# hpy666666/ChineseChessAI

Measured on AMD Instinct MI355X. Metric: self-play games/sec @ 50 MCTS sims, higher is better.
Workload: dtype bf16

## Files before the change

chinesechessai_amd/_lib.py:

```python
import ctypes as C
import os
import subprocess
import sys

_HERE = os.path.dirname(os.path.abspath(__file__))
CSRC = os.path.join(_HERE, "csrc")
LIB_PATH = os.path.join(CSRC, "libxq_hip.so")
SOURCES = [os.path.join(CSRC, "xq_engine.hip"), os.path.join(CSRC, "xq_conv.hip"), os.path.join(CSRC, "xq_replay.hip"),
           os.path.join(CSRC, "xq_tower.hip"), os.path.join(CSRC, "xq_policy.hip")]
HEADERS = [os.path.join(CSRC, "xq_device.hpp"), os.path.join(CSRC, "xq_attack.hpp"), os.path.join(CSRC, "xq_mfma.hpp"), os.path.join(CSRC, "xq_tower_probes.hpp"),
           os.path.join(CSRC, "xq_tower1wa.hpp"), os.path.join(CSRC, "xq_tower1wa_body.inc"), os.path.join(CSRC, "xq_policy_fc1w_body.inc"),
           os.path.join(_HERE, "..", "include", "xq_selfplay.h"), os.path.join(_HERE, "..", "include", "xq_debug.h")]

MAX_MOVES = 128
MAX_PLIES = 70
WINNER_NONE = 2
NO_KING = -1
POLICY_SIZE = 8100
STATE_WORDS = 10
(S_PLAYER, S_MOVE_COUNT, S_WINNER, S_RED_KING, S_BLACK_KING, S_NO_CAPTURE, S_CONSEC_CHECKS, S_REASON,
 S_REASON_SIDE, S_REASON_COUNT) = range(10)
EVAL_PRIORS, EVAL_LOGITS_F32, EVAL_LOGITS_BF16 = 0, 1, 2
PLANES_NONE, PLANES_NCHW_F32, PLANES_NCHW_BF16, PLANES_NHWC16_BF16 = 0, 1, 2, 3
SAMPLE_RECORD_BYTES = 48 + 8 + 4 + 4 + 256 + 256
# ... 98 lines not shown
                                     C.c_void_p, C.c_void_p, C.c_void_p]),
    "xq_engine_create": (C.c_int, [C.POINTER(Config), C.POINTER(C.c_void_p)]),
    "xq_engine_destroy": (None, [C.c_void_p]),
    "xq_engine_set_stream": (C.c_int, [C.c_void_p, C.c_void_p]),
    "xq_engine_set_pow_table": (C.c_int, [C.c_void_p, C.c_void_p, C.c_int]),
    "xq_engine_new_games": (C.c_int, [C.c_void_p, C.c_void_p]),
    "xq_engine_set_logit_columns": (C.c_int, [C.c_void_p, C.c_void_p, C.c_int]),
    "xq_engine_set_temperature": (C.c_int, [C.c_void_p, C.c_double, C.c_void_p, C.c_int]),
    "xq_engine_set_root_noise": (C.c_int, [C.c_void_p, C.c_double, C.c_double, C.c_uint64]),
    "xq_engine_set_tree_reuse": (C.c_int, [C.c_void_p, C.c_int]),
    "xq_engine_set_virtual_loss": (C.c_int, [C.c_void_p, C.c_int]),
    "xq_engine_leaf_slots": (C.c_int, [C.c_void_p]),
    "xq_engine_tree_stats": (C.c_int, [C.c_void_p, C.c_void_p, C.c_void_p]),
    "xq_engine_read_root_priors": (C.c_int, [C.c_void_p, C.c_void_p]),
    "xq_engine_set_uniforms": (C.c_int, [C.c_void_p, C.c_void_p]),
    "xq_engine_set_roots": (C.c_int, [C.c_void_p, C.c_void_p, C.c_void_p]),
    "xq_engine_search_round": (C.c_int, [C.c_void_p, C.c_int, C.c_int, C.c_void_p, C.c_void_p, C.c_void_p]),
    "xq_engine_eval_hashnet": (C.c_int, [C.c_void_p, C.c_int]),
    "xq_engine_end_search": (C.c_int, [C.c_void_p, C.c_int, C.c_void_p, C.c_void_p]),
    "xq_engine_play_move": (C.c_int, [C.c_void_p]),
    "xq_engine_finalize": (C.c_int, [C.c_void_p]),
    "xq_engine_active_games": (C.c_int, [C.c_void_p, C.c_void_p]),
    "xq_engine_active_games_post": (C.c_int, [C.c_void_p]),
    "xq_engine_active_games_poll": (C.c_int, [C.c_void_p, C.c_void_p, C.c_void_p]),
    "xq_engine_priors_ptr": (C.c_void_p, [C.c_void_p]),
    "xq_engine_values_ptr": (C.c_void_p, [C.c_void_p]),
    "xq_engine_rounds_per_move": (C.c_int, [C.c_void_p]),
    "xq_engine_read_leaves": (C.c_int, [C.c_void_p] * 6),
    "xq_engine_write_priors": (C.c_int, [C.c_void_p] * 3),
    "xq_engine_read_root_visits": (C.c_int, [C.c_void_p] * 4),
    "xq_engine_read_tree": (C.c_int, [C.c_void_p, C.c_int, C.c_int] + [C.c_void_p] * 8),
    "xq_engine_read_games": (C.c_int, [C.c_void_p] * 8),
    "xq_engine_read_samples": (C.c_int, [C.c_void_p] * 9),
    "xq_engine_pack_samples": (C.c_int, [C.c_void_p, C.c_void_p]),
    "xq_engine_set_root_eval_carry": (C.c_int, [C.c_void_p, C.c_int]),
    "xq_engine_roots_not_ready": (C.c_int, [C.c_void_p, C.c_void_p]),
    "xq_engine_set_row_compaction": (C.c_int, [C.c_void_p, C.c_int]),
    "xq_engine_set_leaf_dedupe": (C.c_int, [C.c_void_p, C.c_int]),
    "xq_engine_set_eval_cache": (C.c_int, [C.c_void_p, C.c_int]),
    "xq_engine_eval_cache_stats": (C.c_int, [C.c_void_p, C.c_void_p, C.c_int]),
    "xq_engine_row_map": (C.c_int, [C.c_void_p, C.POINTER(C.c_void_p), C.POINTER(C.c_void_p)]),
    "xq_engine_read_row_history": (C.c_int, [C.c_void_p, C.c_void_p, C.c_int, C.POINTER(C.c_int64), C.c_int]),
    "xq_engine_read_leaf_rows": (C.c_int, [C.c_void_p, C.c_void_p]),
    "xq_engine_refill_begin": (C.c_int, [C.c_void_p, C.c_void_p, C.c_int]),
    "xq_engine_refill_step": (C.c_int, [C.c_void_p, C.c_void_p, C.c_void_p]),
    "xq_engine_refill_read_games": (C.c_int, [C.c_void_p] * 8),
    "xq_engine_refill_read_slots": (C.c_int, [C.c_void_p, C.c_void_p]),
    "xq_engine_set_pairing": (C.c_int, [C.c_void_p, C.c_void_p]),
    "xq_engine_refill_begin2": (C.c_int, [C.c_void_p, C.c_void_p, C.c_int, C.c_void_p]),
    "xq_engine_search_round2": (C.c_int, [C.c_void_p, C.c_int, C.c_int, C.c_void_p, C.c_void_p, C.c_int, C.c_void_p, C.c_void_p,
                                          C.c_void_p]),
    "xq_engine_end_search2": (C.c_int, [C.c_void_p, C.c_int, C.c_void_p, C.c_void_p, C.c_int, C.c_void_p, C.c_void_p]),
    "xq_engine_row_map_net": (C.c_int, [C.c_void_p, C.c_int, C.POINTER(C.c_void_p), C.POINTER(C.c_void_p)]),
    "xq_engine_read_row_history_net": (C.c_int, [C.c_void_p, C.c_int, C.c_void_p, C.c_int, C.POINTER(C.c_int64), C.c_int]),
    "xq_engine_eval_hashnet2": (C.c_int, [C.c_void_p, C.c_int, C.c_int]),
    "xq_engine_set_per_slot_reuse": (C.c_int, [C.c_void_p, C.c_int, C.c_int]),
    "xq_conv3x3_nhwc_bf16": (C.c_int, [C.c_void_p, C.c_void_p, C.c_void_p, C.c_void_p, C.c_void_p, C.c_void_p,
                                       C.c_int, C.c_int, C.c_int]),
    "xq_heads_nhwc_bf16": (C.c_int, [C.c_void_p] * 6 + [C.c_int]),
    "xq_tower_nhwc_bf16": (C.c_int, [C.c_void_p] * 9 + [C.c_int, C.c_int, C.c_void_p, C.c_void_p]),
    "xq_policy_fc_bf16": (C.c_int, [C.c_void_p] * 5 + [C.c_int, C.c_int, C.c_int, C.c_void_p]),
    "xq_value_head_bf16": (C.c_int, [C.c_void_p] * 7 + [C.c_int, C.c_void_p]),
    "xq_replay_last_error": (C.c_char_p, []),
    "xq_replay_create": (C.c_int, [C.c_int, C.c_int64, C.POINTER(C.c_void_p)]),
    "xq_replay_destroy": (None, [C.c_void_p]),
    "xq_replay_size": (C.c_int64, [C.c_void_p]),
    "xq_replay_push_records": (C.c_int, [C.c_void_p, C.c_void_p, C.c_void_p, C.c_int, C.c_void_p]),
    "xq_replay_encode_batch": (C.c_int, [C.c_void_p, C.c_void_p, C.c_void_p, C.c_int, C.c_void_p, C.c_void_p]),
    "xq_replay_read_records": (C.c_int, [C.c_void_p, C.c_void_p, C.c_void_p, C.c_int, C.c_void_p]),
    "xq_engine_profile": (C.c_int, [C.c_void_p, C.c_int]),
    "xq_engine_profile_read": (C.c_int, [C.c_void_p] * 5),
}

_DEBUG_SIGNATURES = {
    "xq_tower_set_variant": (None, [C.c_int]),
    "xq_tower_set_clock_sample": (None, [C.c_void_p]),
    "xq_tower_debug_stamps": (C.c_int, [C.c_void_p] * 9 + [C.c_int, C.c_int, C.c_void_p]),
    "xq_mfma_probe": (C.c_int, [C.c_void_p] * 4 + [C.c_int, C.c_int, C.c_int]),
    "xq_conv3x3_set_variant": (None, [C.c_int]),
    "xq_conv3x3_debug_stamps": (C.c_int, [C.c_int, C.c_int] + [C.c_void_p] * 6 + [C.c_int, C.c_int, C.c_void_p]),
    "xq_engine_set_search_occupancy": (None, [C.c_int]),
    "xq_engine_set_search_stamps": (C.c_int, [C.c_void_p]),
    "xq_policy_fc_set_variant": (None, [C.c_int]),
    "xq_policy_fc_debug_stamps": (C.c_int, [C.c_int, C.c_void_p, C.c_void_p, C.c_void_p, C.c_void_p, C.c_void_p, C.c_int, C.c_int, C.c_int, C.c_void_p]),
    "xq_policy_fc_debug": (C.c_int, [C.c_int] + [C.c_void_p] * 5 + [C.c_int, C.c_int, C.c_int]),
}

EXPORTS = sorted(_SIGNATURES)
DEBUG_EXPORTS = sorted(_DEBUG_SIGNATURES)
ROW_HISTORY = 65536


def lib():
    global _lib
    if _lib is None:
        if not os.path.exists(LIB_PATH):
            try:
                build()
            except Exception as ex:
                raise XqError("libxq_hip.so is not built (%s) and could not be compiled (%s): run "
                              "`python -c 'import __graft_entry__ as g; g.build()'`; the HIP path has no CPU fallback"
                              % (LIB_PATH, ex))
        _preload_torch_hip_runtime()
        L = C.CDLL(LIB_PATH)
        for table in (_SIGNATURES, _DEBUG_SIGNATURES):
            for name, (res, args) in table.items():
                fn = getattr(L, name)
                fn.restype = res
                fn.argtypes = args
        _lib = L
    return _lib


def check(rc):
    if rc != 0:
        msg = lib().xq_last_error()
        raise XqError("libxq_hip error %d: %s" % (rc, msg.decode() if msg else "?"))


def ptr(a):
    return None if a is None else a.ctypes.data_as(C.c_void_p)
```

chinesechessai_amd/csrc/xq_engine.hip:

```cpp
#include "xq_device.hpp"
#include "../../include/xq_selfplay.h"
#include "../../include/xq_debug.h"
#include <hip/hip_runtime.h>
#include <math.h>
#include <stdio.h>
#include <stdlib.h>
#include <string.h>
#include <string>
#include <thread>
#include <vector>

using namespace xq;

struct __align__(16) GameS {
    int8_t  side;
    uint8_t move_count;
    int8_t  winner;
    uint8_t reason;
    int8_t  reason_side;
    uint8_t reason_count;
    int8_t  rk, bk;
    uint8_t nocap, cchk, n_hist, n_root;
    uint8_t done, n_samples, error, n_plies;
};
// ... 1083 lines not shown
                    if (lane == 0) E.leaf_side[slot] = (int8_t)leaf_side;
                    if (lane == 1) E.leaf_net[slot] = (uint8_t)net;
                }
                if (planes) write_planes(bd, leaf_side, planes, fmt, slot);
            };
            const MoveResult mr = wave_make_move<false, true>(L.bd, st, L.path_move[depth - 1], hist, L.maps, L.cand, L.legal, L.own_sq,
                                                              early, E.want_check != 0);
            flags |= mr.is_check ? F_CHECK : 0;
            XQ_STAMP(7);
            const bool terminal = (mr.n_legal == 0) || (st.winner != WINNER_NONE);
            if (!terminal) {
                if (lane == 0) {
                    T.fl[node] = (uint8_t)flags;
                    E.leaf_node[slot] = (uint16_t)node; E.leaf_mult[slot] = (uint8_t)sims_left; E.leaf_n[slot] = (uint8_t)mr.n_legal;
                    E.leaf_depth[slot] = (uint8_t)depth;
                }
                for (int j = lane; j < mr.n_legal; j += 64) E.leaf_moves[(size_t)slot * MAXM + j] = L.legal[j];
                if (lane < depth) E.leaf_path[(size_t)slot * PATH_CAP + lane] = L.path_node[lane];
                if (depth > 64 && lane + 64 < depth) E.leaf_path[(size_t)slot * PATH_CAP + 64 + lane] = L.path_node[lane + 64];
                if (STAMP && lane == 0) stp[8] = __builtin_amdgcn_s_memtime();
                const uint32_t bdw = lane < 12 ? pack_dword(L.bd, lane) : 0u;
                int ec = -1;
                if (E.ec_on) {
                    ec = eval_cache_probe(E, h, bdw, leaf_side, net, ec_first, true, E.dedupe && (unsigned)(look.ent >> 32) == E.dd_tag);
                    if (lane == 0) E.leaf_ec[slot] = ec;
                }
                if (E.dedupe && (ec < 0 || E.ec_on == 2)) dedupe_finish(E, slot, bdw, leaf_side, look, net);
                if (STAMP && lane == 0) stp[9] = __builtin_amdgcn_s_memtime();
                return;
            }
            flags |= F_TERM;
            if (st.winner == st.side) flags |= F_VAL_POS;
            else if (st.winner == -st.side) flags |= F_VAL_NEG;
            if (lane == 0) T.fl[node] = (uint8_t)flags;
        }
        const double v = (flags & F_VAL_POS) ? 1.0 : ((flags & F_VAL_NEG) ? -1.0 : 0.0);
        backup(T, root, L.path_node, depth, v, 1);
        sims_left--;
    }
}

template <int OCC, bool VL, bool STAMP = false>
__global__ __launch_bounds__(64, OCC) void k_search_round(Eng E, int round, int batch_count, EvalPair ev, void *planes, int fmt,
                                                          unsigned long long *stamps = nullptr)
{
    __shared__ WaveLds L;
    if constexpr (VL) search_round_generic<true>(E, L, round, batch_count, ev, planes, fmt);
    else search_round_one<STAMP>(E, L, round, batch_count, ev, planes, fmt, stamps);
}

__constant__ uint32_t c_crc_table[256];

__device__ __forceinline__ uint32_t crc_byte(uint32_t crc, uint32_t b)
{
    return c_crc_table[(crc ^ b) & 0xffu] ^ (crc >> 8);
}

__global__ __launch_bounds__(64) void k_hashnet(Eng E, int salt0, int salt1)
{
    __shared__ WaveLds L;
    const int g = blockIdx.x, lane = XQ_LANE;
    if (E.gs[g / E.leaf_slots].done || E.leaf_node[g] == LEAF_NONE) return;
    unpack_to_lds(E.leaf_board + (size_t)g * 12, L.bd);
    wave_sync();
    const int salt = E.leaf_net[g] ? salt1 : salt0;
    uint32_t crc = 0xffffffffu;
    for (int s = 0; s < 90; s++) crc = crc_byte(crc, (uint32_t)(uint8_t)L.bd[s]);
    crc = crc_byte(crc, (uint32_t)(uint8_t)E.leaf_side[g]);
    if (salt) crc = crc_byte(crc, (uint32_t)salt & 0xffu);
    const uint32_t h0 = ~crc;
    const int n = E.leaf_n[g];
    for (int j = lane; j < n; j += 64) {
        const int mv = E.leaf_moves[(size_t)g * MAXM + j], from = mv / 90, to = mv % 90;
        uint32_t c = ~h0;
        c = crc_byte(c, from / 9); c = crc_byte(c, from % 9); c = crc_byte(c, to / 9); c = crc_byte(c, to % 9);
        const uint32_t h = ~c;
        E.priors[(size_t)g * MAXM + j] = (float)((h >> 8) % 64u + 1u) / 1024.0f;
    }
    if (lane == 0) E.values[g] = ((double)((h0 >> 4) % 65u) - 32.0) / 64.0;
}

constexpr int ROW_HIST = 65536;

__global__ __launch_bounds__(1024) void k_assign_rows(Eng E, int n_slots, unsigned seq)
{
    __shared__ int wtot[16];
    const int tid = threadIdx.x, lane = tid & 63, wave = tid >> 6;
    int base = 0, base1 = 0;
    int32_t *const row_src1 = E.row_src + E.n_slots;
    for (int start = 0; start < n_slots; start += 16 * 1024) {
        const int s0 = start + tid * 16;
        uint32_t w[8] = { 0xffffffffu, 0xffffffffu, 0xffffffffu, 0xffffffffu, 0xffffffffu, 0xffffffffu, 0xffffffffu, 0xffffffffu };
        if (s0 + 16 <= n_slots) {
            const uint4 a = *reinterpret_cast<const uint4 *>(E.leaf_node + s0), b = *reinterpret_cast<const uint4 *>(E.leaf_node + s0 + 8);
            w[0] = a.x; w[1] = a.y; w[2] = a.z; w[3] = a.w; w[4] = b.x; w[5] = b.y; w[6] = b.z; w[7] = b.w;
        } else {
            for (int i = 0; i < 16; i++)
                if (s0 + i < n_slots) {
                    const uint32_t v = E.leaf_node[s0 + i];
                    w[i >> 1] = (i & 1) ? (w[i >> 1] & 0x0000ffffu) | (v << 16) : (w[i >> 1] & 0xffff0000u) | v;
                }
        }
        uint32_t flags = 0;
#pragma unroll
        for (int i = 0; i < 16; i++) {
            const uint32_t v = (i & 1) ? w[i >> 1] >> 16 : w[i >> 1] & 0xffffu;
            if (v != LEAF_NONE) flags |= 1u << i;
        }
        if (E.ec_on == 1) {
            uint32_t cached = 0;
            if (s0 + 16 <= n_slots) {
#pragma unroll
                for (int i4 = 0; i4 < 4; i4++) {
                    const int4 c = reinterpret_cast<const int4 *>(E.leaf_ec + s0)[i4];
                    cached |= (c.x >= 0 ? 1u : 0u) << (4 * i4) | (c.y >= 0 ? 2u : 0u) << (4 * i4) | (c.z >= 0 ? 4u : 0u) << (4 * i4) |
                              (c.w >= 0 ? 8u : 0u) << (4 * i4);
                }
            } else {
                for (int i = 0; i < 16; i++)
                    if (s0 + i < n_slots && E.leaf_ec[s0 + i] >= 0) cached |= 1u << i;
            }
            flags &= ~cached;
        }
        uint32_t dups = 0;
        if (E.dedupe) {
            if (s0 + 16 <= n_slots) {
                const uint4 d4 = *reinterpret_cast<const uint4 *>(E.leaf_dup + s0);
                const uint32_t dw[4] = { d4.x, d4.y, d4.z, d4.w };
#pragma unroll
                for (int i = 0; i < 16; i++)
                    if ((dw[i >> 2] >> ((i & 3) * 8)) & 0xffu) dups |= 1u << i;
                if (dups) *reinterpret_cast<uint4 *>(E.leaf_dup + s0) = make_uint4(0, 0, 0, 0);
            } else {
                for (int i = 0; i < 16; i++)
                    if (s0 + i < n_slots && E.leaf_dup[s0 + i]) { dups |= 1u << i; E.leaf_dup[s0 + i] = 0; }
            }
            dups &= flags;
            flags &= ~dups;
        }
        uint32_t net1 = 0;
        if (E.two_net) {
            if (s0 + 16 <= n_slots) {
                const uint4 n4 = *reinterpret_cast<const uint4 *>(E.leaf_net + s0);
                const uint32_t nw[4] = { n4.x, n4.y, n4.z, n4.w };
#pragma unroll
                for (int i = 0; i < 16; i++)
                    if ((nw[i >> 2] >> ((i & 3) * 8)) & 0xffu) net1 |= 1u << i;
            } else {
                for (int i = 0; i < 16; i++)
                    if (s0 + i < n_slots && E.leaf_net[s0 + i]) net1 |= 1u << i;
            }
            net1 &= flags;
        }
        const int mine = __popc(flags & ~net1) | (__popc(net1) << 16);
        int incl = mine;
#pragma unroll
        for (int d = 1; d < 64; d <<= 1) { const int o = __shfl_up(incl, d, 64); if (lane >= d) incl += o; }
        if (lane == 63) wtot[wave] = incl;
        __syncthreads();
        int off = incl - mine, total = 0;
#pragma unroll
        for (int k = 0; k < 16; k++) { const int c = wtot[k]; off += k < wave ? c : 0; total += c; }
        int rows[16];
        int r = base + (off & 0xffff), r1 = base1 + (off >> 16);
#pragma unroll
        for (int i = 0; i < 16; i++) {
            const bool p = (flags >> i) & 1u, n1 = (net1 >> i) & 1u;
            rows[i] = p ? (n1 ? r1 : r) : -1;
            if (p) {
                if (n1) { row_src1[r1] = s0 + i; r1++; }
                else { E.row_src[r] = s0 + i; r++; }
            }
        }
        if (s0 + 16 <= n_slots) {
#pragma unroll
            for (int i = 0; i < 4; i++)
                reinterpret_cast<int4 *>(E.leaf_row + s0)[i] = make_int4(rows[4 * i], rows[4 * i + 1], rows[4 * i + 2], rows[4 * i + 3]);
        } else {
            for (int i = 0; i < 16; i++)
                if (s0 + i < n_slots) E.leaf_row[s0 + i] = rows[i];
        }
        base += total & 0xffff; base1 += total >> 16;
        __syncthreads();
        if (dups) {
            const unsigned *tab_lo = reinterpret_cast<const unsigned *>(E.dd_tab);
#pragma unroll
            for (int i = 0; i < 16; i++)
                if ((dups >> i) & 1u) {
                    const unsigned rep = __hip_atomic_load(&tab_lo[2 * (size_t)(unsigned)E.leaf_pos[s0 + i]], __ATOMIC_RELAXED, __HIP_MEMORY_SCOPE_AGENT);
                    E.leaf_row[s0 + i] = __hip_atomic_load(&E.leaf_row[rep], __ATOMIC_RELAXED, __HIP_MEMORY_SCOPE_AGENT);
                }
        }
    }
    if (tid == 0) {
        E.row_count[0] = base; E.row_count[1] = base1;
        E.row_hist[seq & (ROW_HIST - 1)] = base + base1;
        E.row_hist_net[seq & (ROW_HIST - 1)] = base; E.row_hist_net[ROW_HIST + (seq & (ROW_HIST - 1))] = base1;
    }
}

__global__ __launch_bounds__(64) void k_end_search(Eng E, EvalPair ev)
{
    __shared__ WaveLds L;
    const int g = blockIdx.x;
    const GameS gs = load_gs(E.gs + g);
    if (gs.done) return;
    const Tree T = tree_of(E, g);
    const int root = E.root_node[g];
    if (E.vloss) {
        for (int k = 0; k < E.leaf_slots; k++)
            consume_eval<true>(E, g, g * E.leaf_slots + k, L, T, root, ev, gs.n_plies);
    } else {
        consume_eval<false>(E, g, g, L, T, root, ev, gs.n_plies);
    }
}

__device__ double np_sum(const double *a, int n)
{
    if (n < 8) {
        double res = 0.;
        for (int i = 0; i < n; i++) res += a[i];
        return res;
    }
    double r0 = a[0], r1 = a[1], r2 = a[2], r3 = a[3], r4 = a[4], r5 = a[5], r6 = a[6], r7 = a[7];
    int i;
    for (i = 8; i < n - (n % 8); i += 8) {
        r0 += a[i]; r1 += a[i + 1]; r2 += a[i + 2]; r3 += a[i + 3];
        r4 += a[i + 4]; r5 += a[i + 5]; r6 += a[i + 6]; r7 += a[i + 7];
    }
    double res = ((r0 + r1) + (r2 + r3)) + ((r4 + r5) + (r6 + r7));
    for (; i < n; i++) res += a[i];
    return res;
}

__global__ __launch_bounds__(64) void k_play_move(Eng E)
{
    __shared__ WaveLds L;
    const int g = blockIdx.x, lane = XQ_LANE;
    GameS gs = load_gs(E.gs + g);
    if (gs.done) return;
    const Tree T = tree_of(E, g);
    const int root = E.root_node[g];
    const int nc = T.nc[root], first = T.first[root];
    if (nc == 0) { gs.done = 1; store_gs(E.gs + g, gs); return; }

    for (int j = lane; j < nc; j += 64) L.ibuf[j] = (int)T.N[first + j];
    unpack_to_lds(E.board + (size_t)g * 12, L.bd);
    wave_sync();

    const int pair_v = uni((int)E.pairing[g]);
    const bool store = (gs.side == 1) || pair_v == 0;
    if (store) {
        const size_t si = (size_t)g * XQ_MAX_PLIES + gs.n_samples;
        if (lane < 12) E.s_board[si * 12 + lane] = E.board[(size_t)g * 12 + lane];
        for (int j = lane; j < MAXM; j += 64) {
            E.s_moves[si * MAXM + j] = j < nc ? T.mv[first + j] : 0;
            E.s_counts[si * MAXM + j] = j < nc ? (uint16_t)L.ibuf[j] : 0;
        }
        if (lane == 0) { E.s_player[si] = gs.side; E.s_n[si] = (uint8_t)nc; }
    }

    int pick = -1;
    if (lane == 0) {
        if (E.temperature < 0.01) {
            int am = 0;
            for (int j = 1; j < nc; j++) if (L.ibuf[j] > L.ibuf[am]) am = j;
            for (int j = 0; j < nc; j++) L.fbuf[j] = 0.0;
            L.fbuf[am] = 1.0;
        } else {
            for (int j = 0; j < nc; j++) {
                const int c = L.ibuf[j];
                L.fbuf[j] = (E.pow_table && c < E.pow_n) ? E.pow_table[c] : (double)c;
            }
            const double sum = np_sum(L.fbuf, nc);
// ... 898 lines not shown
    return 0;
}

static int g_search_occ = 4;
extern "C" void xq_engine_set_search_occupancy(int waves_per_simd) { g_search_occ = waves_per_simd; }
#if XQ_TOWER_PROBES
static void *g_search_stamps = nullptr;
#endif
extern "C" int xq_engine_set_search_stamps(void *dev_u64x16_per_game)
{
#if XQ_TOWER_PROBES
    g_search_stamps = dev_u64x16_per_game;
    return 0;
#else
    (void)dev_u64x16_per_game;
    return XQ_E_INVALID;
#endif
}

static int two_net_ok(xq_engine *e)
{
    if (e->slot_reuse) return 0;
    if (e->E.ec_on || e->ec_want) return fail(XQ_E_INVALID, "a two-network round cannot use the evaluation cache (two networks answer differently for one position): xq_engine_set_eval_cache(e, 0)");
    if (e->E.eval_carry) return fail(XQ_E_INVALID, "a two-network round cannot use the root evaluation carry-over (the carried priors are the mover's network's)");
    return 0;
}

static int search_round_impl(xq_engine *e, int round, int eval_kind, const void *ev_a, const void *ev_v, int eval_kind1,
                             const void *ev_a1, const void *ev_v1, void *planes, int two)
{
    if (!e) return fail(XQ_E_INVALID, "null engine");
    if (round < 0 || round >= e->E.nrounds) return fail(XQ_E_INVALID, "round out of range");
    if (eval_kind < XQ_EVAL_PRIORS || eval_kind > XQ_EVAL_LOGITS_BF16) return fail(XQ_E_INVALID, "bad eval_kind");
    if (eval_kind1 < XQ_EVAL_PRIORS || eval_kind1 > XQ_EVAL_LOGITS_BF16) return fail(XQ_E_INVALID, "bad eval_kind");
    if (round > 0 && (!ev_a || !ev_v || !ev_a1 || !ev_v1)) return fail(XQ_E_INVALID, "evaluator output missing");
    if (two) { if (int rc = two_net_ok(e)) return rc; }
    if (eval_kind1 != XQ_EVAL_PRIORS && ev_a1 && e->E.compact && !e->row_map_fetched)
        return fail(XQ_E_INVALID, "logits handed in by slot while row compaction is on: fetch xq_engine_row_map_net (rows are compacted)");
    e->E.two_net = two ? 1 : 0;
    if (!planes_ok(e->cfg.planes_format)) return fail(XQ_E_INVALID, "bad planes_format");
    if (eval_kind != XQ_EVAL_PRIORS && ev_a && e->E.compact && !e->row_map_fetched)
        return fail(XQ_E_INVALID, "logits handed in by slot while row compaction is on: fetch xq_engine_row_map (rows are compacted) "
                                  "or switch xq_engine_set_row_compaction off");
    HIPCHK(hipSetDevice(e->cfg.device));
    const int start = round * e->E.leaf_batch;
    const int batch = (start + e->E.leaf_batch <= e->E.sims) ? e->E.leaf_batch : e->E.sims - start;
    std::pair<hipEvent_t, hipEvent_t> *ev = nullptr;
    if (e->prof && (e->prof_seen++ % (unsigned)e->prof) == 0) {
        if (e->ev_search_used >= 4096) { if (int rc = drain_events(e)) return rc; }
        ev = next_events(e->ev_search, e->ev_search_used);
        if (ev) HIPCHK(hipEventRecord(ev->first, e->stream));
    }
    const int fmt = planes ? e->cfg.planes_format : XQ_PLANES_NONE;
    const EvalPair evp{ { { ev_a, ev_v, eval_kind, 0 }, { ev_a1, ev_v1, eval_kind1, 0 } } };
    e->E.ec_epoch = e->ec_epoch; e->E.ec_seq = ++e->ec_seq;
    if (e->E.dedupe) {
        if (++e->dd_tag == 0) {
            HIPCHK(hipMemsetAsync(e->E.dd_tab, 0, ((size_t)e->E.dd_mask + 1) * 8, e->stream));
            e->dd_tag = 1;
        }
        e->E.dd_tag = e->dd_tag;
    }
#define XQ_LAUNCH_SEARCH(OCC, VLB) hipLaunchKernelGGL((k_search_round<OCC, VLB>), dim3(e->E.G), dim3(64), 0, e->stream, e->E, \
                                                    round, batch, evp, planes, fmt, (unsigned long long *)nullptr)
    if (e->E.vloss) XQ_LAUNCH_SEARCH(4, true);
#if XQ_TOWER_PROBES
    else if (g_search_stamps)
        hipLaunchKernelGGL((k_search_round<4, false, true>), dim3(e->E.G), dim3(64), 0, e->stream, e->E, round, batch, evp,
                           planes, fmt, (unsigned long long *)g_search_stamps);
#endif
    else switch (g_search_occ) {
#if XQ_TOWER_PROBES
    case 3: XQ_LAUNCH_SEARCH(3, false); break;
    case 5: XQ_LAUNCH_SEARCH(5, false); break;
    case 6: XQ_LAUNCH_SEARCH(6, false); break;
    case 8: XQ_LAUNCH_SEARCH(8, false); break;
#endif
    default: XQ_LAUNCH_SEARCH(4, false); break;
    }
#undef XQ_LAUNCH_SEARCH
    HIPCHK(hipGetLastError());
    if (ev) HIPCHK(hipEventRecord(ev->second, e->stream));
    if (e->E.compact) {
        hipLaunchKernelGGL(k_assign_rows, dim3(1), dim3(1024), 0, e->stream, e->E, e->E.G * e->E.leaf_slots, e->row_seq);
        HIPCHK(hipGetLastError());
        e->row_seq++;
    }
    return 0;
}

extern "C" int xq_engine_search_round(xq_engine *e, int round, int eval_kind, const void *ev_a, const void *ev_v,
                                      void *planes)
{
    return search_round_impl(e, round, eval_kind, ev_a, ev_v, eval_kind, ev_a, ev_v, planes, 0);
}

extern "C" int xq_engine_search_round2(xq_engine *e, int round, int eval_kind0, const void *ev_a0, const void *ev_v0,
                                       int eval_kind1, const void *ev_a1, const void *ev_v1, void *planes)
{
    return search_round_impl(e, round, eval_kind0, ev_a0, ev_v0, eval_kind1, ev_a1, ev_v1, planes, 1);
}

extern "C" int xq_engine_set_row_compaction(xq_engine *e, int enable)
{
    if (!e) return fail(XQ_E_INVALID, "null engine");
    if ((enable ? 1 : 0) != e->E.compact) e->row_map_fetched = false;
    e->E.compact = enable ? 1 : 0;
    if (!enable) e->E.dedupe = 0;
    return 0;
}

extern "C" int xq_engine_set_leaf_dedupe(xq_engine *e, int enable)
{
    if (!e) return fail(XQ_E_INVALID, "null engine");
    if (enable && !e->E.compact) return fail(XQ_E_INVALID, "leaf dedupe needs row compaction (xq_engine_set_row_compaction)");
    e->E.dedupe = enable ? 1 : 0;
    return 0;
}

extern "C" int xq_engine_set_eval_cache(xq_engine *e, int log2_entries)
{
    if (!e) return fail(XQ_E_INVALID, "null engine");
    const bool verify = log2_entries < 0;
    if (verify) log2_entries = -log2_entries;
    if (log2_entries == 0) { e->ec_want = 0; eval_cache_apply(e); return 0; }
    if (log2_entries < 10 || log2_entries > 24) return fail(XQ_E_INVALID, "eval cache: 10 <= log2_entries <= 24");
    HIPCHK(hipSetDevice(e->cfg.device));
    const size_t n = (size_t)1 << log2_entries;
    if (!e->E.ec_state || (size_t)e->E.ec_mask + 1 != n) {
        HIPCHK(hipStreamSynchronize(e->stream));
        int bad = dalloc(e, e->E.ec_state, n);
        bad |= dalloc(e, e->E.ec_key, n * 16); bad |= dalloc(e, e->E.ec_prior, n * MAXM);
        if (!e->E.leaf_ec) bad |= dalloc(e, e->E.leaf_ec, (size_t)e->E.G * 64);
        if (!e->E.ec_stats) bad |= dalloc(e, e->E.ec_stats, (size_t)3 * e->E.G * 64);
        if (bad) return fail(XQ_E_HIP, "hipMalloc failed for the evaluation cache");
        HIPCHK(hipMemsetAsync(e->E.leaf_ec, 0xff, (size_t)e->E.G * 64 * 4, e->stream));
        e->E.ec_mask = (int)(n - 1);
    }
    eval_cache_age_out(e);
    e->ec_want = verify ? 2 : 1;
    eval_cache_apply(e);
    e->E.ec_stat_stride = e->E.G * 64;
    return 0;
}

extern "C" int xq_engine_eval_cache_stats(xq_engine *e, uint64_t *hits_fills_host , int reset)
{
    if (!e || !hits_fills_host) return fail(XQ_E_INVALID, "null argument");
    hits_fills_host[0] = hits_fills_host[1] = hits_fills_host[2] = 0;
    if (!e->E.ec_stats) return 0;
    HIPCHK(hipSetDevice(e->cfg.device));
    const size_t stride = (size_t)e->E.G * 64, slots = (size_t)e->E.G * (size_t)e->E.leaf_slots;
    std::vector<uint32_t> h(slots);
    for (int k = 0; k < 3; k++) {
        HIPCHK(hipMemcpyAsync(h.data(), e->E.ec_stats + k * stride, slots * 4, hipMemcpyDeviceToHost, e->stream));
        HIPCHK(hipStreamSynchronize(e->stream));
        for (size_t i = 0; i < slots; i++) hits_fills_host[k] += h[i];
        if (reset) HIPCHK(hipMemsetAsync(e->E.ec_stats + k * stride, 0, slots * 4, e->stream));
    }
    return 0;
}

extern "C" int xq_engine_row_map_net(xq_engine *e, int net, const int32_t **row_src_dev, const int32_t **row_count_dev)
{
    if (!e || !row_src_dev || !row_count_dev) return fail(XQ_E_INVALID, "null argument");
    if (net < 0 || net > 1) return fail(XQ_E_INVALID, "net must be 0 or 1");
    e->row_map_fetched = true;
// ... 490 lines not shown
```

chinesechessai_amd/csrc/xq_policy.hip:

```cpp
#include "../../include/xq_selfplay.h"
#include "../../include/xq_debug.h"
#include "xq_mfma.hpp"
#include <atomic>
#include <type_traits>

#ifndef XQ_TOWER_PROBES
#define XQ_TOWER_PROBES 0
#endif

namespace {
using namespace xqm;

constexpr int BM = 256, BN = 192;
constexpr int A_BYTES = BM * 128, W_BYTES = BN * 128, STAGE_BYTES = A_BYTES + W_BYTES;
constexpr int FC_LDS_BYTES = 2 * STAGE_BYTES;

struct FcArgs {
    const uint16_t *act;
    const uint16_t *w;
    const float *bias;
    uint16_t *out;
    int M, N, K, ncol;
    const int32_t *n_rows;
    unsigned long long *stamps;
// ... 144 lines not shown
template <int ABL = 0>
__global__ __launch_bounds__(256, 1) void k_policy_fc1w(FcArgs P)
{
    const int tid = threadIdx.x, lane = tid & 63;
    const int wave = __builtin_amdgcn_readfirstlane(tid >> 6);
    const int wm = wave >> 1, wn = wave & 1;
    const int r16 = lane & 15, q = lane >> 4;
    const int nwg = gridDim.x, orig = blockIdx.x, xcd = orig & 7, qd = nwg >> 3, rem = nwg & 7;
    const int t = (xcd < rem ? xcd * (qd + 1) : rem * (qd + 1) + (xcd - rem) * qd) + (orig >> 3);
    const int rb = t / P.ncol, cb = t - rb * P.ncol;
    const int m0 = rb * BM, n0 = cb * BN;
    int M = P.M;
    if (P.n_rows) { const int n = *P.n_rows; M = n < M ? n : M; }
    if (m0 >= M) return;
    const int rows = M - m0 < BM ? M - m0 : BM;
    const int K2 = P.K * 2, N2 = P.N * 2, nst = P.K >> 6;
    const uint16_t *act_t = P.act + (size_t)m0 * P.K;
    const uint16_t *w_t = P.w + (size_t)n0 * P.K;
    uint16_t *out_t = P.out + (size_t)m0 * P.N + n0;
    const float *bias_t = P.bias + n0;
    const int act_bytes = rows * K2, w_bytes = BN * K2;
    const int gr = (r16 >> 1) & 7;
    const int vfa = (wn * 96 + 8 * (r16 >> 2) + (r16 & 3)) * 128 + ((q ^ gr) << 4);
    const int vfb = (wm * 128 + r16) * 128 + ((q ^ gr) << 4);
    const int ga = 4 * (wave & 1) + ((lane >> 4) & 3), gw = 2 * wave + ((lane >> 4) & 1);
    const int vdma = (lane >> 3) * K2 + (((lane & 7) ^ ga) << 4);
    const int vdmaw = (lane >> 3) * K2 + (((lane & 7) ^ gw) << 4);
    const int vstore = ((wm * 128 + r16) * P.N + wn * 96 + 8 * q) * 2;
    const int vrow = wm * 128 + r16;
    const int vbias = (wn * 96 + 8 * q) * 4;
    unsigned long long *stamp_p = ABL >= 7 ? P.stamps + (size_t)blockIdx.x * 32 : nullptr;
#if XQ_TOWER_PROBES
    if constexpr (ABL == 7) { XQ_FC1W_ASM(XQ_FC1W_BODY_STAMPED); return; }
    if constexpr (ABL == 8) { XQ_FC1W_ASM(XQ_FC1W_BODY_NODMA_STAMPED); return; }
    if constexpr (ABL == 2) { XQ_FC1W_ASM(XQ_FC1W_BODY_FRONT); return; }
    if constexpr (ABL == 3) { XQ_FC1W_ASM(XQ_FC1W_BODY_NODMA); return; }
    if constexpr (ABL == 4) { XQ_FC1W_ASM(XQ_FC1W_BODY_NOMFMA); return; }
    if constexpr (ABL == 5) { XQ_FC1W_ASM(XQ_FC1W_BODY_EVEN); return; }
    if constexpr (ABL == 6) { XQ_FC1W_ASM(XQ_FC1W_BODY_NOMFMA_NOLDS); return; }
#endif
    XQ_FC1W_ASM(XQ_FC1W_BODY);
}

__global__ __launch_bounds__(256) void k_value_head(const uint16_t *__restrict__ hv, const uint16_t *__restrict__ w1,
                                                    const float *__restrict__ b1, const float *__restrict__ w2,
                                                    const float *__restrict__ b2, uint16_t *__restrict__ out, int M,
                                                    const int32_t *__restrict__ n_rows)
{
    constexpr int K = 720, KP = 736;
    if (n_rows) { const int n = *n_rows; M = n < M ? n : M; }
    const int lane = threadIdx.x & 63, r16 = lane & 15, q = lane >> 4;
    const int row0 = (blockIdx.x * 4 + (threadIdx.x >> 6)) * 16;
    if (row0 >= M) return;
    const int row = row0 + r16 < M ? row0 + r16 : M - 1;
    const uint16_t *xr = hv + (size_t)row * K + q * 8;
    const uint16_t *wr = w1 + (size_t)r16 * KP + q * 8;
    f32x4 acc[8];
#pragma unroll
    for (int nt = 0; nt < 8; nt++) acc[nt] = *reinterpret_cast<const f32x4 *>(b1 + nt * 16 + 4 * q);
#pragma unroll 1
    for (int ks = 0; ks < KP / 32; ks++) {
        const bf16x8 x = *reinterpret_cast<const bf16x8 *>(xr + ks * 32);
#pragma unroll
        for (int nt = 0; nt < 8; nt++) {
            const bf16x8 w = *reinterpret_cast<const bf16x8 *>(wr + (size_t)nt * 16 * KP + ks * 32);
            acc[nt] = __builtin_amdgcn_mfma_f32_16x16x32_bf16(w, x, acc[nt], 0, 0, 0);
        }
    }
    float part = 0.f;
#pragma unroll
    for (int nt = 0; nt < 8; nt++) {
        const f32x4 c = *reinterpret_cast<const f32x4 *>(w2 + nt * 16 + 4 * q);
#pragma unroll
        for (int i = 0; i < 4; i++) part += fmaxf(acc[nt][i], 0.f) * c[i];
    }
    part += __shfl_xor(part, 16, 64);
    part += __shfl_xor(part, 32, 64);
    if (q == 0 && row0 + r16 < M) {
        const float v = tanhf(part + b2[0]);
        out[row0 + r16] = (uint16_t)(pack_bf16x2(v, 0.f) & 0xffffu);
    }
}

}

static int g_fc_variant = -1;
extern "C" void xq_policy_fc_set_variant(int v) { g_fc_variant = v; }

static int fc_lds_opt_in()
{
    static std::atomic<uint64_t> done{ 0 };
    int dev = 0;
    if (hipGetDevice(&dev) != hipSuccess || dev < 0 || dev >= 64) return XQ_E_HIP;
    if (done.load(std::memory_order_acquire) >> dev & 1) return 0;
    if (hipFuncSetAttribute(reinterpret_cast<const void *>(&k_policy_fc<0>), hipFuncAttributeMaxDynamicSharedMemorySize,
                            FC_LDS_BYTES) != hipSuccess)
        return XQ_E_HIP;
    if (hipFuncSetAttribute(reinterpret_cast<const void *>(&k_policy_fc1w<0>), hipFuncAttributeMaxDynamicSharedMemorySize,
                            XQ_FC1W_LDS_BYTES) != hipSuccess)
        return XQ_E_HIP;
#if XQ_TOWER_PROBES
    if (hipFuncSetAttribute(reinterpret_cast<const void *>(&k_policy_fc1w<2>), hipFuncAttributeMaxDynamicSharedMemorySize, XQ_FC1W_LDS_BYTES) != hipSuccess ||
        hipFuncSetAttribute(reinterpret_cast<const void *>(&k_policy_fc1w<3>), hipFuncAttributeMaxDynamicSharedMemorySize, XQ_FC1W_LDS_BYTES) != hipSuccess ||
        hipFuncSetAttribute(reinterpret_cast<const void *>(&k_policy_fc1w<4>), hipFuncAttributeMaxDynamicSharedMemorySize, XQ_FC1W_LDS_BYTES) != hipSuccess ||
        hipFuncSetAttribute(reinterpret_cast<const void *>(&k_policy_fc1w<5>), hipFuncAttributeMaxDynamicSharedMemorySize, XQ_FC1W_LDS_BYTES) != hipSuccess ||
        hipFuncSetAttribute(reinterpret_cast<const void *>(&k_policy_fc1w<6>), hipFuncAttributeMaxDynamicSharedMemorySize, XQ_FC1W_LDS_BYTES) != hipSuccess ||
        hipFuncSetAttribute(reinterpret_cast<const void *>(&k_policy_fc1w<7>), hipFuncAttributeMaxDynamicSharedMemorySize, XQ_FC1W_LDS_BYTES) != hipSuccess ||
        hipFuncSetAttribute(reinterpret_cast<const void *>(&k_policy_fc1w<8>), hipFuncAttributeMaxDynamicSharedMemorySize, XQ_FC1W_LDS_BYTES) != hipSuccess)
        return XQ_E_HIP;
    if (hipFuncSetAttribute(reinterpret_cast<const void *>(&k_policy_fc<1>), hipFuncAttributeMaxDynamicSharedMemorySize, FC_LDS_BYTES) != hipSuccess ||
        hipFuncSetAttribute(reinterpret_cast<const void *>(&k_policy_fc<2>), hipFuncAttributeMaxDynamicSharedMemorySize, FC_LDS_BYTES) != hipSuccess)
        return XQ_E_HIP;
#endif
    done.fetch_or(1ull << dev, std::memory_order_release);
    return 0;
}

extern "C" int xq_policy_fc_bf16(void *stream, const void *act, const void *w, const void *bias, void *out, int M, int N, int K,
                                 const void *n_rows_dev)
{
    if (!act || !w || !bias || !out || M <= 0 || N <= 0 || K < 64 || (K & 63) || N % BN) return XQ_E_INVALID;
    if (int rc = fc_lds_opt_in()) return rc;
    FcArgs a{ (const uint16_t *)act, (const uint16_t *)w, (const float *)bias, (uint16_t *)out, M, N, K, N / BN,
              (const int32_t *)n_rows_dev, nullptr };
    const int ntiles = ((M + BM - 1) / BM) * (N / BN);
#if XQ_TOWER_PROBES
    if (g_fc_variant >= 2 && g_fc_variant <= 6) {
        const hipStream_t hs = reinterpret_cast<hipStream_t>(stream);
        if (g_fc_variant == 2) hipLaunchKernelGGL(k_policy_fc1w<2>, dim3(ntiles), dim3(256), XQ_FC1W_LDS_BYTES, hs, a);
        if (g_fc_variant == 3) hipLaunchKernelGGL(k_policy_fc1w<3>, dim3(ntiles), dim3(256), XQ_FC1W_LDS_BYTES, hs, a);
        if (g_fc_variant == 4) hipLaunchKernelGGL(k_policy_fc1w<4>, dim3(ntiles), dim3(256), XQ_FC1W_LDS_BYTES, hs, a);
        if (g_fc_variant == 5) hipLaunchKernelGGL(k_policy_fc1w<5>, dim3(ntiles), dim3(256), XQ_FC1W_LDS_BYTES, hs, a);
        if (g_fc_variant == 6) hipLaunchKernelGGL(k_policy_fc1w<6>, dim3(ntiles), dim3(256), XQ_FC1W_LDS_BYTES, hs, a);
        return hipGetLastError() == hipSuccess ? 0 : XQ_E_HIP;
    }
#endif
    if (g_fc_variant > 1) return XQ_E_INVALID;
    if (g_fc_variant != 0)
        hipLaunchKernelGGL(k_policy_fc1w<0>, dim3(ntiles), dim3(256), XQ_FC1W_LDS_BYTES, reinterpret_cast<hipStream_t>(stream), a);
    else
        hipLaunchKernelGGL(k_policy_fc<0>, dim3(ntiles), dim3(512), FC_LDS_BYTES, reinterpret_cast<hipStream_t>(stream), a);
    return hipGetLastError() == hipSuccess ? 0 : XQ_E_HIP;
}

extern "C" int xq_policy_fc_debug(int ablate, void *stream, const void *act, const void *w, const void *bias, void *out, int M, int N,
                                  int K)
{
#if XQ_TOWER_PROBES
    if (!act || !w || !bias || !out || M <= 0 || N <= 0 || K < 64 || (K & 63) || N % BN || ablate < 1 || ablate > 2) return XQ_E_INVALID;
    if (int rc = fc_lds_opt_in()) return rc;
    FcArgs a{ (const uint16_t *)act, (const uint16_t *)w, (const float *)bias, (uint16_t *)out, M, N, K, N / BN, nullptr, nullptr };
    const int ntiles = ((M + BM - 1) / BM) * (N / BN);
    if (ablate == 1) hipLaunchKernelGGL(k_policy_fc<1>, dim3(ntiles), dim3(512), FC_LDS_BYTES, reinterpret_cast<hipStream_t>(stream), a);
    else hipLaunchKernelGGL(k_policy_fc<2>, dim3(ntiles), dim3(512), FC_LDS_BYTES, reinterpret_cast<hipStream_t>(stream), a);
    return hipGetLastError() == hipSuccess ? 0 : XQ_E_HIP;
#else
    return XQ_E_INVALID;
#endif
}

extern "C" int xq_policy_fc_debug_stamps(int nodma, void *stream, const void *act, const void *w, const void *bias, void *out, int M, int N,
                                         int K, void *stamps_dev)
{
#if XQ_TOWER_PROBES
    if (!act || !w || !bias || !out || !stamps_dev || M <= 0 || N <= 0 || K < 64 || (K & 63) || N % BN) return XQ_E_INVALID;
    if (int rc = fc_lds_opt_in()) return rc;
    FcArgs a{ (const uint16_t *)act, (const uint16_t *)w, (const float *)bias, (uint16_t *)out, M, N, K, N / BN, nullptr,
              (unsigned long long *)stamps_dev };
    const int ntiles = ((M + BM - 1) / BM) * (N / BN);
    const hipStream_t hs = reinterpret_cast<hipStream_t>(stream);
    if (nodma) hipLaunchKernelGGL(k_policy_fc1w<8>, dim3(ntiles), dim3(256), XQ_FC1W_LDS_BYTES, hs, a);
    else hipLaunchKernelGGL(k_policy_fc1w<7>, dim3(ntiles), dim3(256), XQ_FC1W_LDS_BYTES, hs, a);
    return hipGetLastError() == hipSuccess ? 0 : XQ_E_HIP;
#else
    return XQ_E_INVALID;
#endif
}

extern "C" int xq_value_head_bf16(void *stream, const void *hv, const void *w1, const void *b1, const void *w2, const void *b2,
                                  void *values, int n_rows, const void *n_rows_dev)
{
    if (!hv || !w1 || !b1 || !w2 || !b2 || !values || n_rows <= 0) return XQ_E_INVALID;
    hipLaunchKernelGGL(k_value_head, dim3((n_rows + 63) / 64), dim3(256), 0, reinterpret_cast<hipStream_t>(stream),
                       (const uint16_t *)hv, (const uint16_t *)w1, (const float *)b1, (const float *)w2, (const float *)b2,
                       (uint16_t *)values, n_rows, (const int32_t *)n_rows_dev);
    return hipGetLastError() == hipSuccess ? 0 : XQ_E_HIP;
}
```

include/xq_debug.h:

```cpp
#ifndef XQ_DEBUG_H
#define XQ_DEBUG_H
#include <stdint.h>

#ifdef __cplusplus
extern "C" {
#endif

void xq_tower_set_variant(int variant);

void xq_tower_set_clock_sample(void *dev_u64x3);

int  xq_tower_debug_stamps(void *hip_stream, const void *planes_dev, const void *w1_dev, const void *wt_dev,
                           const void *bias_dev, const void *wh_dev, const void *bh_dev, void *policy_out_dev,
                           void *value_out_dev, int n_boards, int n_blocks, void *stamps_dev);

int  xq_mfma_probe(void *hip_stream, const void *seed64_dev, const void *weights_dev, void *out_dev, int n_workgroups,
                   int iters, int mode);

void xq_conv3x3_set_variant(int variant);

int  xq_conv3x3_debug_stamps(int variant, int ablate, void *hip_stream, const void *x_dev, const void *w_dev,
                             const void *bias_dev, const void *residual_dev, void *y_dev, int n_boards, int relu,
                             void *stamps_dev);

void xq_policy_fc_set_variant(int variant);

int  xq_policy_fc_debug(int ablate, void *hip_stream, const void *act_dev, const void *w_dev, const void *bias_dev, void *out_dev,
                        int n_rows, int n_cols, int k);

int  xq_policy_fc_debug_stamps(int nodma, void *hip_stream, const void *act_dev, const void *w_dev, const void *bias_dev,
                               void *out_dev, int n_rows, int n_cols, int k, void *stamps_dev);

void xq_engine_set_search_occupancy(int waves_per_simd);

int  xq_engine_set_search_stamps(void *dev_u64x16_per_game);

#ifdef __cplusplus
}
#endif
#endif
```

Before: 13200.

## Specialize row-assignment kernel and add LDS-staged MFMA value head

The row-assignment kernel is templated on the cache, dedupe and two-net flags so the unused branches compile away. It issues all per-slot loads up front and stages row_src writes in a 64 KB LDS buffer so they go out coalesced after a barrier. Duplicate resolution now batches its atomic loads and writes rows back vectorised. Separately, a new value-head kernel DMAs the weights into LDS in slices and runs bf16 MFMA, and it is the default path (variant -1). The large static LDS use limits the single-block kernel, and the new value head depends on fixed K=720 shapes.

```diff
diff --git a/chinesechessai_amd/_lib.py b/chinesechessai_amd/_lib.py
--- a/chinesechessai_amd/_lib.py
+++ b/chinesechessai_amd/_lib.py
@@ -204,6 +204,7 @@
     "xq_engine_set_search_occupancy": (None, [C.c_int]),
     "xq_engine_set_search_stamps": (C.c_int, [C.c_void_p]),
     "xq_policy_fc_set_variant": (None, [C.c_int]),
+    "xq_value_head_set_variant": (None, [C.c_int]),
     "xq_policy_fc_debug_stamps": (C.c_int, [C.c_int, C.c_void_p, C.c_void_p, C.c_void_p, C.c_void_p, C.c_void_p, C.c_int, C.c_int, C.c_int, C.c_void_p]),
     "xq_policy_fc_debug": (C.c_int, [C.c_int] + [C.c_void_p] * 5 + [C.c_int, C.c_int, C.c_int]),
 }
diff --git a/chinesechessai_amd/csrc/xq_engine.hip b/chinesechessai_amd/csrc/xq_engine.hip
--- a/chinesechessai_amd/csrc/xq_engine.hip
+++ b/chinesechessai_amd/csrc/xq_engine.hip
@@ -1189,17 +1189,28 @@
 
 constexpr int ROW_HIST = 65536;
 
+template <bool EC, bool DD, bool TN>
 __global__ __launch_bounds__(1024) void k_assign_rows(Eng E, int n_slots, unsigned seq)
 {
     __shared__ int wtot[16];
+    __shared__ int srcl[16 * 1024];
     const int tid = threadIdx.x, lane = tid & 63, wave = tid >> 6;
     int base = 0, base1 = 0;
     int32_t *const row_src1 = E.row_src + E.n_slots;
     for (int start = 0; start < n_slots; start += 16 * 1024) {
         const int s0 = start + tid * 16;
         uint32_t w[8] = { 0xffffffffu, 0xffffffffu, 0xffffffffu, 0xffffffffu, 0xffffffffu, 0xffffffffu, 0xffffffffu, 0xffffffffu };
-        if (s0 + 16 <= n_slots) {
+        const bool full = s0 + 16 <= n_slots;
+        int4 ec4[4] = { make_int4(-1, -1, -1, -1), make_int4(-1, -1, -1, -1), make_int4(-1, -1, -1, -1), make_int4(-1, -1, -1, -1) };
+        uint4 d4 = make_uint4(0, 0, 0, 0), n4 = make_uint4(0, 0, 0, 0);
+        if (full) {
             const uint4 a = *reinterpret_cast<const uint4 *>(E.leaf_node + s0), b = *reinterpret_cast<const uint4 *>(E.leaf_node + s0 + 8);
+            if (EC) {
+#pragma unroll
+                for (int i4 = 0; i4 < 4; i4++) ec4[i4] = reinterpret_cast<const int4 *>(E.leaf_ec + s0)[i4];
+            }
+            if (DD) d4 = *reinterpret_cast<const uint4 *>(E.leaf_dup + s0);
+            if (TN) n4 = *reinterpret_cast<const uint4 *>(E.leaf_net + s0);
             w[0] = a.x; w[1] = a.y; w[2] = a.z; w[3] = a.w; w[4] = b.x; w[5] = b.y; w[6] = b.z; w[7] = b.w;
         } else {
             for (int i = 0; i < 16; i++)
@@ -1214,12 +1225,12 @@
             const uint32_t v = (i & 1) ? w[i >> 1] >> 16 : w[i >> 1] & 0xffffu;
             if (v != LEAF_NONE) flags |= 1u << i;
         }
-        if (E.ec_on == 1) {
+        if (EC) {
             uint32_t cached = 0;
-            if (s0 + 16 <= n_slots) {
+            if (full) {
 #pragma unroll
                 for (int i4 = 0; i4 < 4; i4++) {
-                    const int4 c = reinterpret_cast<const int4 *>(E.leaf_ec + s0)[i4];
+                    const int4 c = ec4[i4];
                     cached |= (c.x >= 0 ? 1u : 0u) << (4 * i4) | (c.y >= 0 ? 2u : 0u) << (4 * i4) | (c.z >= 0 ? 4u : 0u) << (4 * i4) |
                               (c.w >= 0 ? 8u : 0u) << (4 * i4);
                 }
@@ -1230,9 +1241,8 @@
             flags &= ~cached;
         }
         uint32_t dups = 0;
-        if (E.dedupe) {
-            if (s0 + 16 <= n_slots) {
-                const uint4 d4 = *reinterpret_cast<const uint4 *>(E.leaf_dup + s0);
+        if (DD) {
+            if (full) {
                 const uint32_t dw[4] = { d4.x, d4.y, d4.z, d4.w };
 #pragma unroll
                 for (int i = 0; i < 16; i++)
@@ -1245,10 +1255,22 @@
             dups &= flags;
             flags &= ~dups;
         }
+        int32_t pos[16] = { 0, 0, 0, 0, 0, 0, 0, 0, 0, 0, 0, 0, 0, 0, 0, 0 };
+        if (dups) {
+            if (full) {
+#pragma unroll
+                for (int i4 = 0; i4 < 4; i4++) {
+                    const int4 p4 = reinterpret_cast<const int4 *>(E.leaf_pos + s0)[i4];
+                    pos[4 * i4] = p4.x; pos[4 * i4 + 1] = p4.y; pos[4 * i4 + 2] = p4.z; pos[4 * i4 + 3] = p4.w;
+                }
+            } else {
+                for (int i = 0; i < 16; i++)
+                    if ((dups >> i) & 1u) pos[i] = E.leaf_pos[s0 + i];
+            }
+        }
         uint32_t net1 = 0;
-        if (E.two_net) {
-            if (s0 + 16 <= n_slots) {
-                const uint4 n4 = *reinterpret_cast<const uint4 *>(E.leaf_net + s0);
+        if (TN) {
+            if (full) {
                 const uint32_t nw[4] = { n4.x, n4.y, n4.z, n4.w };
 #pragma unroll
                 for (int i = 0; i < 16; i++)
@@ -1269,34 +1291,53 @@
 #pragma unroll
         for (int k = 0; k < 16; k++) { const int c = wtot[k]; off += k < wave ? c : 0; total += c; }
         int rows[16];
-        int r = base + (off & 0xffff), r1 = base1 + (off >> 16);
+        const int cnt0 = total & 0xffff, cnt1 = total >> 16;
+        int l0 = off & 0xffff, l1 = cnt0 + (off >> 16);
 #pragma unroll
         for (int i = 0; i < 16; i++) {
             const bool p = (flags >> i) & 1u, n1 = (net1 >> i) & 1u;
-            rows[i] = p ? (n1 ? r1 : r) : -1;
+            rows[i] = p ? (n1 ? base1 + l1 - cnt0 : base + l0) : -1;
             if (p) {
-                if (n1) { row_src1[r1] = s0 + i; r1++; }
-                else { E.row_src[r] = s0 + i; r++; }
-            }
-        }
-        if (s0 + 16 <= n_slots) {
+                if (n1) { srcl[l1] = s0 + i; l1++; }
+                else { srcl[l0] = s0 + i; l0++; }
+            }
+        }
+        if (full) {
+            if (!dups || flags) {
 #pragma unroll
-            for (int i = 0; i < 4; i++)
-                reinterpret_cast<int4 *>(E.leaf_row + s0)[i] = make_int4(rows[4 * i], rows[4 * i + 1], rows[4 * i + 2], rows[4 * i + 3]);
+                for (int i = 0; i < 4; i++)
+                    reinterpret_cast<int4 *>(E.leaf_row + s0)[i] = make_int4(rows[4 * i], rows[4 * i + 1], rows[4 * i + 2], rows[4 * i + 3]);
+            }
         } else {
             for (int i = 0; i < 16; i++)
                 if (s0 + i < n_slots) E.leaf_row[s0 + i] = rows[i];
         }
-        base += total & 0xffff; base1 += total >> 16;
         __syncthreads();
+        for (int j = tid; j < cnt0; j += 1024) E.row_src[base + j] = srcl[j];
+        for (int j = tid; j < cnt1; j += 1024) row_src1[base1 + j] = srcl[cnt0 + j];
+        base += cnt0; base1 += cnt1;
         if (dups) {
             const unsigned *tab_lo = reinterpret_cast<const unsigned *>(E.dd_tab);
+            unsigned rep[16];
+            int32_t rrow[16];
 #pragma unroll
             for (int i = 0; i < 16; i++)
-                if ((dups >> i) & 1u) {
-                    const unsigned rep = __hip_atomic_load(&tab_lo[2 * (size_t)(unsigned)E.leaf_pos[s0 + i]], __ATOMIC_RELAXED, __HIP_MEMORY_SCOPE_AGENT);
-                    E.leaf_row[s0 + i] = __hip_atomic_load(&E.leaf_row[rep], __ATOMIC_RELAXED, __HIP_MEMORY_SCOPE_AGENT);
-                }
+                rep[i] = __hip_atomic_load(&tab_lo[((dups >> i) & 1u) ? 2 * (size_t)(unsigned)pos[i] : 0], __ATOMIC_RELAXED, __HIP_MEMORY_SCOPE_AGENT);
+#pragma unroll
+            for (int i = 0; i < 16; i++)
+                rrow[i] = __hip_atomic_load(&E.leaf_row[((dups >> i) & 1u) ? rep[i] : 0u], __ATOMIC_RELAXED, __HIP_MEMORY_SCOPE_AGENT);
+            if (full) {
+#pragma unroll
+                for (int i = 0; i < 16; i++)
+                    if ((dups >> i) & 1u) rows[i] = rrow[i];
+#pragma unroll
+                for (int i = 0; i < 4; i++)
+                    reinterpret_cast<int4 *>(E.leaf_row + s0)[i] = make_int4(rows[4 * i], rows[4 * i + 1], rows[4 * i + 2], rows[4 * i + 3]);
+            } else {
+#pragma unroll
+                for (int i = 0; i < 16; i++)
+                    if ((dups >> i) & 1u) E.leaf_row[s0 + i] = rrow[i];
+            }
         }
     }
     if (tid == 0) {
@@ -2361,7 +2402,15 @@
     HIPCHK(hipGetLastError());
     if (ev) HIPCHK(hipEventRecord(ev->second, e->stream));
     if (e->E.compact) {
-        hipLaunchKernelGGL(k_assign_rows, dim3(1), dim3(1024), 0, e->stream, e->E, e->E.G * e->E.leaf_slots, e->row_seq);
+        {
+            using assign_fn = void (*)(Eng, int, unsigned);
+            static const assign_fn fn[8] = { k_assign_rows<false, false, false>, k_assign_rows<true, false, false>,
+                                             k_assign_rows<false, true, false>,  k_assign_rows<true, true, false>,
+                                             k_assign_rows<false, false, true>,  k_assign_rows<true, false, true>,
+                                             k_assign_rows<false, true, true>,   k_assign_rows<true, true, true> };
+            const int which = (e->E.ec_on == 1 ? 1 : 0) | (e->E.dedupe ? 2 : 0) | (e->E.two_net ? 4 : 0);
+            hipLaunchKernelGGL(fn[which], dim3(1), dim3(1024), 0, e->stream, e->E, e->E.G * e->E.leaf_slots, e->row_seq);
+        }
         HIPCHK(hipGetLastError());
         e->row_seq++;
     }
diff --git a/chinesechessai_amd/csrc/xq_policy.hip b/chinesechessai_amd/csrc/xq_policy.hip
--- a/chinesechessai_amd/csrc/xq_policy.hip
+++ b/chinesechessai_amd/csrc/xq_policy.hip
@@ -250,6 +250,99 @@
     }
 }
 
+constexpr int VH_SLICE_BYTES = 128 * 256;
+constexpr int VH_LDS_BYTES = 5 * VH_SLICE_BYTES;
+
+template <int N> __device__ __forceinline__ void vh_wait_slice()
+{
+    __builtin_amdgcn_sched_barrier(0);
+    __builtin_amdgcn_s_waitcnt(0x0F70 | (N & 15) | ((N >> 4) << 14));
+    __builtin_amdgcn_s_barrier();
+    __builtin_amdgcn_sched_barrier(0);
+}
+
+__global__ __launch_bounds__(256, 1) void k_value_head_lds(const uint16_t *__restrict__ hv, const uint16_t *__restrict__ w1,
+                                                        const float *__restrict__ b1, const float *__restrict__ w2,
+                                                        const float *__restrict__ b2, uint16_t *__restrict__ out, int M,
+                                                        const int32_t *__restrict__ n_rows)
+{
+    constexpr int K = 720, KP = 736, NKS = KP / 32, ROWB = KP * 2;
+    if (n_rows) { const int n = *n_rows; M = n < M ? n : M; }
+    if ((int)blockIdx.x * 64 >= M) return;
+    const int lane = threadIdx.x & 63, r16 = lane & 15, q = lane >> 4;
+    const int wave = __builtin_amdgcn_readfirstlane(threadIdx.x >> 6);
+    const int row0 = (blockIdx.x * 4 + wave) * 16;
+    const int row = row0 + r16 < M ? row0 + r16 : M - 1;
+    const uint16_t *xr = hv + (size_t)row * K + q * 8;
+    f32x4 acc[8];
+#pragma unroll
+    for (int nt = 0; nt < 8; nt++) acc[nt] = *reinterpret_cast<const f32x4 *>(b1 + nt * 16 + 4 * q);
+    bf16x8 x[NKS];
+#pragma unroll
+    for (int ks = 0; ks < NKS; ks++) x[ks] = *reinterpret_cast<const bf16x8 *>(xr + ks * 32);
+
+    const rsrc_t rw = make_rsrc(w1, 128 * ROWB);
+    const int voff = (lane >> 4) * ROWB + (((lane & 15) ^ (wave * 4 + (lane >> 4))) << 4);
+    auto slice_dma = [&](int s, int slot) {
+#pragma unroll
+        for (int j = 0; j < 8; j++) {
+            const int p = j * 4 + wave;
+            dma16_buf_abs(rw, voff, p * 4 * ROWB + s * 256, slot * VH_SLICE_BYTES + p * 1024);
+        }
+    };
+    __builtin_amdgcn_sched_barrier(0);
+#pragma unroll
+    for (int s = 0; s < 5; s++) slice_dma(s, s);
+    __builtin_amdgcn_sched_barrier(0);
+
+    const int fbase = r16 * 256;
+    bf16x8 fw[2][8];
+    auto slice_mfma = [&](int s, int slot, int nk) {
+#pragma unroll
+        for (int nt = 0; nt < 8; nt++) fw[0][nt] = lds_ld128(slot * VH_SLICE_BYTES + nt * 4096 + fbase + ((q ^ r16) << 4));
+        __builtin_amdgcn_sched_group_barrier(0x100, 8, 0);
+#pragma unroll
+        for (int kk = 0; kk < nk; kk++)
+#pragma unroll
+            for (int nt = 0; nt < 8; nt++) {
+                if (kk + 1 < nk) {
+                    fw[(kk + 1) & 1][nt] = lds_ld128(slot * VH_SLICE_BYTES + nt * 4096 + fbase + ((((kk + 1) * 4 + q) ^ r16) << 4));
+                    __builtin_amdgcn_sched_group_barrier(0x100, 1, 0);
+                }
+                acc[nt] = __builtin_amdgcn_mfma_f32_16x16x32_bf16(fw[kk & 1][nt], x[s * 4 + kk], acc[nt], 0, 0, 0);
+                __builtin_amdgcn_sched_group_barrier(0x008, 1, 0);
+            }
+    };
+    vh_wait_slice<32>();
+    slice_mfma(0, 0, 4);
+    vh_wait_slice<24>();
+    slice_dma(5, 0);
+    __builtin_amdgcn_sched_barrier(0);
+    slice_mfma(1, 1, 4);
+    vh_wait_slice<24>();
+    slice_mfma(2, 2, 4);
+    vh_wait_slice<16>();
+    slice_mfma(3, 3, 4);
+    vh_wait_slice<8>();
+    slice_mfma(4, 4, 4);
+    vh_wait_slice<0>();
+    slice_mfma(5, 0, NKS - 20);
+
+    float part = 0.f;
+#pragma unroll
+    for (int nt = 0; nt < 8; nt++) {
+        const f32x4 c = *reinterpret_cast<const f32x4 *>(w2 + nt * 16 + 4 * q);
+#pragma unroll
+        for (int i = 0; i < 4; i++) part += fmaxf(acc[nt][i], 0.f) * c[i];
+    }
+    part += __shfl_xor(part, 16, 64);
+    part += __shfl_xor(part, 32, 64);
+    if (q == 0 && row0 + r16 < M) {
+        const float v = tanhf(part + b2[0]);
+        out[row0 + r16] = (uint16_t)(pack_bf16x2(v, 0.f) & 0xffffu);
+    }
+}
+
 }
 
 static int g_fc_variant = -1;
@@ -345,12 +438,36 @@
 #endif
 }
 
+static int g_vh_variant = -1;
+extern "C" void xq_value_head_set_variant(int v) { g_vh_variant = v; }
+
+static int vh_lds_opt_in()
+{
+    static std::atomic<uint64_t> done{ 0 };
+    int dev = 0;
+    if (hipGetDevice(&dev) != hipSuccess || dev < 0 || dev >= 64) return XQ_E_HIP;
+    if (done.load(std::memory_order_acquire) >> dev & 1) return 0;
+    if (hipFuncSetAttribute(reinterpret_cast<const void *>(&k_value_head_lds), hipFuncAttributeMaxDynamicSharedMemorySize,
+                            VH_LDS_BYTES) != hipSuccess)
+        return XQ_E_HIP;
+    done.fetch_or(1ull << dev, std::memory_order_release);
+    return 0;
+}
+
 extern "C" int xq_value_head_bf16(void *stream, const void *hv, const void *w1, const void *b1, const void *w2, const void *b2,
                                   void *values, int n_rows, const void *n_rows_dev)
 {
     if (!hv || !w1 || !b1 || !w2 || !b2 || !values || n_rows <= 0) return XQ_E_INVALID;
-    hipLaunchKernelGGL(k_value_head, dim3((n_rows + 63) / 64), dim3(256), 0, reinterpret_cast<hipStream_t>(stream),
-                       (const uint16_t *)hv, (const uint16_t *)w1, (const float *)b1, (const float *)w2, (const float *)b2,
-                       (uint16_t *)values, n_rows, (const int32_t *)n_rows_dev);
+    if (g_vh_variant > 1) return XQ_E_INVALID;
+    if (g_vh_variant != 0) {
+        if (int rc = vh_lds_opt_in()) return rc;
+        hipLaunchKernelGGL(k_value_head_lds, dim3((n_rows + 63) / 64), dim3(256), VH_LDS_BYTES, reinterpret_cast<hipStream_t>(stream),
+                           (const uint16_t *)hv, (const uint16_t *)w1, (const float *)b1, (const float *)w2, (const float *)b2,
+                           (uint16_t *)values, n_rows, (const int32_t *)n_rows_dev);
+    } else {
+        hipLaunchKernelGGL(k_value_head, dim3((n_rows + 63) / 64), dim3(256), 0, reinterpret_cast<hipStream_t>(stream),
+                           (const uint16_t *)hv, (const uint16_t *)w1, (const float *)b1, (const float *)w2, (const float *)b2,
+                           (uint16_t *)values, n_rows, (const int32_t *)n_rows_dev);
+    }
     return hipGetLastError() == hipSuccess ? 0 : XQ_E_HIP;
 }
diff --git a/include/xq_debug.h b/include/xq_debug.h
--- a/include/xq_debug.h
+++ b/include/xq_debug.h
@@ -31,6 +31,8 @@
 int  xq_policy_fc_debug_stamps(int nodma, void *hip_stream, const void *act_dev, const void *w_dev, const void *bias_dev,
                                void *out_dev, int n_rows, int n_cols, int k, void *stamps_dev);
 
+void xq_value_head_set_variant(int variant);
+
 void xq_engine_set_search_occupancy(int waves_per_simd);
 
 int  xq_engine_set_search_stamps(void *dev_u64x16_per_game);
```

Result: no change. 13280 (median of 6 runs) (+0.6%).
